# dscripka/openWakeWord

Measured on AMD Instinct MI355X. Metric: real-time audio frames/sec (80 ms frame, 3 wakewords), whole job; real-time streams = value/12.5, higher is better.
Workload: dtype f32 as 3xf16 split MFMA, fp32 accumulate; 1 GPU; 131072 concurrent 16 kHz streams per GPU x 3 heads (alexa,hey_mycroft,hey_jarvis), 80 ms frames, BASELINE configs[3] per-GPU shard; streams_per_gpu=131072, frame_samples=1280, collective=none, gather=none, rccl_ranks=0, pcm_distribution=Gaussian, RMS 3000, pcm=resident in HBM, kernels=mfma_rr_f16x3, graph=False, vad=off, weights=synthetic seed 1234, step_blocks=1

## Files before the change

### openwakeword_amd/csrc/owwhip.hip

```cpp
#include <hip/hip_runtime.h>

#include <algorithm>
#include <cmath>
#include <cstdio>
#include <cstdlib>
#include <cstring>
#include <ctime>
#include <exception>
#include <mutex>
#include <new>
#include <unordered_map>
#include <dlfcn.h>
#include <string>
#include <vector>

#include "owwhip.h"
#include "owwhip_pack.h"
#include "owwhip_ingest.h"
#include "owwhip_mem.h"
#include "owwhip_kernels.h"
#include "owwhip_rr.h"
#include "owwhip_hx.h"
#include "owwhip_vad.h"
#include "owwhip_fused.h"
// ... 90 lines not shown
int stream_create_raw(hipStream_t* s, unsigned flags) { return hipStreamCreateWithFlags(s, flags); }
int stream_destroy_raw(hipStream_t s) { return hipStreamDestroy(s); }
}

namespace {
inline hipError_t herr(int e) { return static_cast<hipError_t>(e); }

hipError_t guard_copy(void* dst, const void* src, size_t n, hipMemcpyKind kind, hipStream_t st) {
    PinnedBuf<char> pin;
    hipError_t e = herr(pin.alloc(n, hipHostMallocDefault));
    if (e != hipSuccess) return e;
    if (kind == hipMemcpyHostToDevice) {
        memcpy(pin, src, n);
        e = hipMemcpyAsync(dst, pin, n, kind, st);
        if (e == hipSuccess) e = hipStreamSynchronize(st);
    } else {
        e = hipMemcpyAsync(pin, src, n, kind, st);
        if (e == hipSuccess) e = hipStreamSynchronize(st);
        if (e == hipSuccess) memcpy(dst, pin, n);
    }
    return e;
}
inline hipError_t copy_async(void* dst, const void* src, size_t n, hipMemcpyKind kind, hipStream_t st) {
    if (guard_mode() && n && (kind == hipMemcpyHostToDevice || kind == hipMemcpyDeviceToHost)) return guard_copy(dst, src, n, kind, st);
    return hipMemcpyAsync(dst, src, n, kind, st);
}
inline hipError_t copy_sync(void* dst, const void* src, size_t n, hipMemcpyKind kind) {
    if (guard_mode() && n && (kind == hipMemcpyHostToDevice || kind == hipMemcpyDeviceToHost)) return guard_copy(dst, src, n, kind, nullptr);
    const hipError_t e = hipMemcpy(dst, src, n, kind);
    return e != hipSuccess || kind != hipMemcpyHostToDevice ? e : hipStreamSynchronize(nullptr);
}

constexpr int kSmallLaunchWgs = 2 * 256;

struct FastGroup : HeadGroup {
    DevBuf<NetDesc> d_nets;
    const float* d_w1pk = nullptr;
    const float* d_b1cat = nullptr;
    const float* d_w1hx = nullptr;
    std::vector<owh::HeadHxNet> hx_net;
};

owh::HeadHxNet make_hx_net(const NetHost& n, int ht, const HxNetPack& p, const float* img, const float* b3, int hx_efeat) {
    const int HP = 16 * ht;
    const float* pd = img + p.pad;
    owh::HeadHxNet o{};
    o.w2hx = img + p.w2; o.b1 = pd; o.ln1g = pd + HP; o.ln1b = pd + 2 * HP; o.b2 = pd + 3 * HP; o.ln2g = pd + 4 * HP; o.ln2b = pd + 5 * HP;
    if (ht == 4) { o.w3 = pd + 6 * HP; o.b3 = b3 ? b3 : pd + 7 * HP; }
    else { o.b3 = pd + 6 * HP; o.w3hx = img + p.w3; o.u3 = std::ldexp(1.0f, -p.e3); }
    o.has_ln = n.has_ln; o.role = n.role; o.head = n.head; o.out_col = n.out_col;
    o.hidden = n.hidden; o.inv_hidden = 1.0f / (float)n.hidden;
    o.u1 = std::ldexp(1.0f, -(hx_efeat + p.e1) + (n.has_ln ? 0 : p.eh)); o.u2 = std::ldexp(1.0f, -(p.e2 + p.eh));
    o.n_out = n.n_out; o.final_act = n.final_act;
    return o;
}

struct EventRec { owm::Event a, b; int cls = 0; };

}

struct oww_ctx : PackIn {
    owm::Stream stream, up_stream, down_stream;
    oww_config cfg{};
    int S = 0, Spad = 0, kmax = 1, TR = 16, NL = 0;
    bool committed = false;
    const int* state_len = kStateLenRr;
// ... 36 lines not shown
    DevBuf<long long> d_prof;
    int prof_block = -1;
    DevBuf<uint32_t> d_nfeat, d_npred, d_nvad;
    DevBuf<float> d_vadring, d_vadin; float vad_threshold = 0.f;
    bool vad = false;
    const float *d_vad_hann = nullptr, *d_vad_encw = nullptr, *d_vad_encb = nullptr, *d_vad_lstmw = nullptr, *d_vad_lstmb = nullptr, *d_vad_wd = nullptr;
    float vad_bd = 0.f, vad_gain = 50.f;
    DevBuf<float> d_vadx, d_vadhc, d_vadlast;
    DevBuf<int16_t> d_tail, d_pcm;
    DevBuf<int16_t> d_long;
    DevBuf<float> d_callmax;
    PinnedBuf<int> h_range;
    int* d_range = nullptr;
    DevBuf<char> d_rs;
    std::vector<float> rs_taps;
    struct Ingest {
        bool ready = false, mixed = false;
        owi::Table tab;
        DevBuf<float> d_taps;
        DevBuf<int16_t> d_hist;
        DevBuf<int16_t> d_out;
        DevBuf<char> d_in;
        DevBuf<uint8_t> d_on;
        DevBuf<IngestClass> d_table;
        DevBuf<uint32_t> d_cls;
        DevBuf<int> d_newcls;
    } ing;
    DevBuf<uint8_t> d_on;
    DevBuf<int> d_lists; PinnedBuf<int> h_lists[2]; owm::Event lists_ev[2]; unsigned lists_turn = 0;
    int k_last = 1;
    float hx_absmax[20] = {};
    std::vector<int16_t> cal_user;
    int small_wgs = kSmallLaunchWgs, small_wgs_heads = kSmallLaunchWgs;
    float hx_selftest_err = 0.f, hx_selftest_ref = 0.f, hx_selftest_score_err = 0.f;
    bool fuse = false;
    DevBuf<float> d_verw, d_verb, d_verthr; DevBuf<int> d_verT;
    int ver_stride = 0, n_verifiers = 0;
    std::vector<int> ver_T;
    bool post_in_heads = false;
    DevBuf<float> d_save;
    DevBuf<int> d_ids;
    DevBuf<int> d_patience;
    DevBuf<float> d_threshold;
    int debounce_frames = 0;
    void* comm = nullptr; int comm_rank = 0, comm_world = 1;
    bool timing = false;
    std::vector<EventRec> ev;
    size_t ev_used = 0;
    double t_ms[OWW_N_KERNEL_CLASSES] = {};
    int64_t t_n[OWW_N_KERNEL_CLASSES] = {};
    bool want_graph = false;
    hipGraph_t graph = nullptr;
    hipGraphExec_t graph_exec = nullptr;
    struct BankHead {
        bool live = false;
        int T = 0, hidden = 0, has_ln = 0, ht = 4, patience = 0;
        float threshold = NAN;
        DevBuf<float> d_img;
        size_t w1_bytes = 0;
        owh::BankHeadDev dev{};
    };
    int bank_K = 0, bank_cap = 0;
    std::vector<BankHead> bank;
    std::vector<int> bank_sub;
    DevBuf<int> d_bank_sub, d_bank_idx;
    DevBuf<float> d_bank_raw, d_bank_scores, d_bank_ring;
// ... 106 lines not shown
        p.prof_block = h->prof_block;
    };
    {
        StageParams p{}; fill(p, h->d_xA, h->d_xB, 3, 2, 3);
        Timed t(h, 2);
        hipLaunchKernelGGL((stage_kernel<CfgB, MFMA, false>), dim3((n_active + CfgB::B - 1) / CfgB::B), dim3(CfgB::NT), CfgB::LDS_BYTES, st, p);
    }
    {
        StageParams p{}; fill(p, h->d_xB, h->d_xC, 7, 4, 5);
        Timed t(h, 3);
        hipLaunchKernelGGL((stage_kernel<CfgC, MFMA, false>), dim3((n_active + CfgC::B - 1) / CfgC::B), dim3(CfgC::NT), CfgC::LDS_BYTES, st, p);
    }
    {
        StageParams p{}; fill(p, h->d_xC, h->d_xD, 11, 6, 7);
        Timed t(h, 4);
        hipLaunchKernelGGL((stage_kernel<CfgD, MFMA, false>), dim3((n_active + CfgD::B - 1) / CfgD::B), dim3(CfgD::NT), CfgD::LDS_BYTES, st, p);
    }
    {
        StageParams p{}; fill(p, h->d_xD, nullptr, 15, 8, 9);
        p.hist19 = h->d_state[10]; p.w19 = h->d_conv[19]; p.feat = h->d_feat; p.emb = h->d_emb; p.nfeat = h->d_nfeat; p.TR = h->TR;
        p.dbg_off[4] = dbg_off[19];
        Timed t(h, 5);
        hipLaunchKernelGGL((stage_kernel<CfgE, MFMA, true>), dim3((n_active + CfgE::B - 1) / CfgE::B), dim3(CfgE::NT), CfgE::LDS_BYTES, st, p);
    }
    HIPCHK(hipGetLastError());
    return 0;
}

template <class CR, class CH, int WG, bool LAST, bool DBG, bool HX>
void launch_rstage(oww_ctx* h, const owr::RStageParams& p, int cls) {
    hipStream_t st = h->stream;
    Timed t(h, cls);
    const int nwg = (p.n_groups + WG - 1) / WG;
    if (HX && !DBG && nwg <= h->small_wgs) hipLaunchKernelGGL((owh::hstage_kernel<CH, LAST, false, WG, 3>), dim3(nwg), dim3(64 * WG), 0, st, p);
    else if (HX) hipLaunchKernelGGL((owh::hstage_kernel<CH, LAST, DBG, WG>), dim3(nwg), dim3(64 * WG), 0, st, p);
    else hipLaunchKernelGGL((owr::rstage_kernel<CR, LAST, DBG>), dim3((p.n_groups + 3) / 4), dim3(256), 0, st, p);
}

template <bool DBG, bool HX>
int run_cnn_rr(oww_ctx* h, const StepArgs& a, int n_active, int mel_stride, int mel_off) {
    using namespace owr;
    hipStream_t st = h->stream;
    int off = 0, dbg_off[20];
    for (int l = 0; l < 20; ++l) { dbg_off[l] = off; off += kLayerOut[l][0] * kLayerOut[l][1] * kLayerOut[l][2]; }
    {
        RAParams p{};
        p.mel = a.mel ? a.mel : h->d_mel; p.mel_stride = mel_stride; p.mel_off = mel_off;
        p.hist_mel = h->d_state[0]; p.hist2 = h->d_state[1];
        p.w0 = h->d_conv[0]; p.w1 = h->d_conv[1]; p.w2 = h->d_conv[2];
        for (int i = 0; i < 3; ++i) { p.scale[i] = h->d_scale[i]; p.shift[i] = h->d_shift[i]; p.dbg_off[i] = dbg_off[i]; }
        p.xout = h->d_xA; p.n_streams = n_active; p.S = h->Spad;
        p.dbg = DBG ? h->d_dbg : nullptr; p.dbg_stride = DBG_FLOATS;
        for (int i = 0; i < 3; ++i) { p.clampv[i] = -0.4f * ldexpf(1.f, h->hx_e[i]); p.dbg_mul[i] = ldexpf(1.f, -h->hx_e[i]); }
        p.xmul = ldexpf(1.f, h->hx_xexp[0]);
        p.range_flag = HX ? h->d_range : nullptr;
        p.stream_on = a.on;
        const int grid = std::min((n_active + 3) / 4, 768);
        Timed t(h, 1);
        if (HX && a.fused_pcm) {
            owf::MelAParams q{};
            q.a = p; q.a.mel = nullptr; q.a.n_streams = h->S;
            q.pcm = a.fused_pcm; q.tail = h->d_tail; q.nfeat = h->d_nfeat; q.hann = h->d_hann; q.mel_start = h->d_mstart; q.mel_taps = h->d_taps; q.mel_off = h->d_meloff; q.mel_dst = h->d_meldst;
            q.mel_out = h->cfg.debug_layers ? h->d_mel : nullptr;
            const int per_cu = std::max(1, std::min(12 / owf::FA_WG, 163840 / owf::FA_LDS_BYTES));
            const int g2 = std::max(1, std::min((q.a.n_streams + owf::FA_WG - 1) / owf::FA_WG, 256 * per_cu));
            hipLaunchKernelGGL(owf::hmelA_kernel<DBG>, dim3(g2), dim3(64 * owf::FA_WG), owf::FA_LDS_BYTES, st, q);
// ... 880 lines not shown
    if (int rc = dalloc(h->stream, h->d_ring, SP * std::max(h->NL, 1) * OWW_SCORE_RING)) return rc;
    if (int rc = dalloc(h->stream, h->d_featinit, (size_t)h->TR * 96)) return rc;
    if (int rc = dalloc(h->stream, h->d_nfeat, SP)) return rc;
    if (int rc = dalloc(h->stream, h->d_npred, SP)) return rc;
    if (int rc = dalloc(h->stream, h->d_vadring, SP * 8)) return rc;
    if (int rc = dalloc(h->stream, h->d_nvad, SP)) return rc;
    if (int rc = dalloc(h->stream, h->d_vadin, SP)) return rc;
    if (h->vad) {
        const size_t G = (SP + 15) / 16;
        if (int rc = dalloc(h->stream, h->d_vadx, G * 4 * 1024)) return rc;
        if (int rc = dalloc(h->stream, h->d_vadhc, G * 4096)) return rc;
        if (int rc = dalloc(h->stream, h->d_vadlast, SP)) return rc;
    }
    if (int rc = dalloc(h->stream, h->d_tail, SP * 480)) return rc;
    if (int rc = dalloc(h->stream, h->d_pcm, (size_t)h->S * OWW_CHUNK * h->kmax)) return rc;
    if (int rc = dalloc(h->stream, h->d_patience, (size_t)std::max(h->NL, 1))) return rc;
    if (int rc = dalloc(h->stream, h->d_threshold, (size_t)std::max(h->NL, 1))) return rc;
    {
        std::vector<float> nanv(std::max(h->NL, 1), NAN);
        HIPCHK(copy_async(h->d_threshold, nanv.data(), nanv.size() * sizeof(float), hipMemcpyHostToDevice, h->stream));
    }
    if (h->cfg.debug_layers) if (int rc = dalloc(h->stream, h->d_dbg, SP * DBG_FLOATS)) return rc;
    if (const char* e = getenv("OWW_PROF_BLOCK")) { h->prof_block = atoi(e); if (int rc = dalloc(h->stream, h->d_prof, (size_t)4 * 256)) return rc; }
    return 0;
}

int set_kernel_lds(oww_ctx* h) {
    int rc = 0;
    auto lds = [&rc](auto kernel, int bytes) { if (!rc) rc = set_lds(kernel, bytes); };
    for (const auto& g : h->groups) if (g.ht == 4) lds(heads64_kernel, heads_lds_bytes(g.NH));
    if (!h->rnn_nets.empty()) lds(heads_rnn_kernel<RNN_SPW>, (int)rnn_lds_bytes(RNN_TMAX));
    if (h->vad) lds(owv::vad_front_kernel, owv::V_LDS_BYTES);
    lds(owf::hmelA_kernel<false>, owf::FA_LDS_BYTES); lds(owf::hmelA_kernel<true>, owf::FA_LDS_BYTES);
    lds(stageA_kernel<true>, CfgA::LDS_BYTES); lds(stageA_kernel<false>, CfgA::LDS_BYTES);
    lds(stage_kernel<CfgB, true, false>, CfgB::LDS_BYTES); lds(stage_kernel<CfgB, false, false>, CfgB::LDS_BYTES);
    lds(stage_kernel<CfgC, true, false>, CfgC::LDS_BYTES); lds(stage_kernel<CfgC, false, false>, CfgC::LDS_BYTES);
    lds(stage_kernel<CfgD, true, false>, CfgD::LDS_BYTES); lds(stage_kernel<CfgD, false, false>, CfgD::LDS_BYTES);
    lds(stage_kernel<CfgE, true, true>, CfgE::LDS_BYTES); lds(stage_kernel<CfgE, false, true>, CfgE::LDS_BYTES);
    return rc;
}

int derive_reset_state(oww_ctx* h, const HxCalib& cal, CommitClock& clk) {
    const size_t SP = h->Spad;
    const int warm = std::min<int>(32, (int)SP);
    hipLaunchKernelGGL(fill_kernel, dim3((warm * 256 + 255) / 256), dim3(256), 0, h->stream, h->d_mel, (size_t)warm * 256, 1.0f);
    const StepArgs args{};
    for (int it = 0; it < 12; ++it)
        if (int rc = run_cnn(h, args, warm, 256, 0)) return rc;
    for (int a = 0; a < N_STATE; ++a)
        HIPCHK(copy_async(h->d_tmpl[a], h->d_state[a], (size_t)h->state_len[a] * (h->rr ? kStateSpgRr[a] : 1) * sizeof(float),
                              hipMemcpyDeviceToDevice, h->stream));
    HIPCHK(hipMemsetAsync(h->d_mel, 0, SP * 8 * h->kmax * 32 * sizeof(float), h->stream));
    HIPCHK(hipMemsetAsync(h->d_emb, 0, SP * 96 * sizeof(float), h->stream));
    if (int rc = do_reset(h, nullptr, (int)SP, nullptr)) return rc;
    HIPCHK(hipStreamSynchronize(h->stream));
    clk.lap("warm-up + reset");
    if (int rc = range_check(h, "oww_commit")) return rc;
    if (h->hx && !getenv("OWW_NO_COMMIT_SELFTEST")) {
        if (int rc = selftest_hx(h, cal)) return rc;
        HIPCHK(hipMemsetAsync(h->d_mel, 0, SP * 8 * h->kmax * 32 * sizeof(float), h->stream));
        HIPCHK(hipMemsetAsync(h->d_emb, 0, SP * 96 * sizeof(float), h->stream));
        HIPCHK(hipMemsetAsync(h->d_raw, 0, SP * std::max(h->NL, 1) * sizeof(float), h->stream));
        if (int rc = do_reset(h, nullptr, (int)SP, nullptr)) return rc;
        HIPCHK(hipStreamSynchronize(h->stream));
        clk.lap("self-test replay + reset");
    }
// ... 344 lines not shown
    if (int rc = build_nets(*h, h->NL, h->TR, h->generic_hmax)) return rc;
    if (h->evt_rows > h->TR)
        return fail(OWW_EINVAL, "oww_events_configure: feature_rows = %d exceeds the handle's feature ring (%d rows)", h->evt_rows, h->TR);
    CommitClock clk(h->hx ? "f16-split" : "family");
    HxCalib cal;
    if (h->hx) {
        if (int rc = calibrate_hx(h, cal)) return rc;
        h->probe_emb = cal.ref_emb; h->probe_nb = cal.nb;
        clk.lap("calibration (total)");
        if (getenv("OWW_DEBUG_CALIB"))
            for (int l = 0; l < 20; ++l) fprintf(stderr, "calib layer %2d: max|a| %-12.5g e_in %4d e_out %4d\n", l, h->hx_absmax[l], h->hx_ein[l], h->hx_e[l]);
    }
    HostBuf hb;
    WeightOff off;
    HeadGroups hg;
    h->no_wide_heads = getenv("OWW_NO_WIDE_HEADS") != nullptr;
    if (int rc = pack_mel_tables(*h, hb, off)) return rc;
    if (int rc = pack_cnn(*h, hb, off)) return rc;
    pack_net_arrays(*h, hb, off);
    if (int rc = pack_head_groups(*h, hg, hb, off)) return rc;
    h->groups.clear();
    for (const HeadGroup& g : hg.groups) h->groups.push_back(FastGroup{g});
    h->generic_nets = hg.generic_nets; h->rnn_nets = hg.rnn_nets;
    h->vad = !h->vad_blob.empty();
    if (int rc = pack_vad(*h, hb, off, h->vad_gain, h->vad_bd)) return rc;
    clk.lap("weight packing (host)");
    if (int rc = bind_weights(h, hb, off)) return rc;
    if (int rc = alloc_range_flag(h)) return rc;
    clk.lap("weight upload");
    if (int rc = alloc_state(h)) return rc;
    h->fuse = h->hx && !getenv("OWW_NO_FUSE");
    if (const char* e = getenv("OWW_SMALL_WGS")) h->small_wgs = atoi(e);
    if (const char* e = getenv("OWW_SMALL_WGS_HEADS")) h->small_wgs_heads = atoi(e);
    if (const char* e = getenv("OWW_GENERIC_SPW")) { const int v = atoi(e); h->generic_spw = v == 4 || v == 16 ? v : 0; }
    h->post_in_heads = h->fuse && h->groups.size() == 1 && h->groups[0].ht == 4 && h->generic_nets.empty() && h->rnn_nets.empty() && h->NL > 0;
    if (int rc = set_kernel_lds(h)) return rc;
    clk.lap("state allocation");
    if (int rc = derive_reset_state(h, cal, clk)) return rc;
    if (h->bank_K > 0) if (int rc = alloc_bank(h)) return rc;
    if (h->vpool_cap > 0) if (int rc = alloc_verifiers(h)) return rc;
    if (events_on(h)) if (int rc = alloc_events(h)) return rc;
    h->committed = true;
    return OWW_OK;
    OWW_GUARD_END
}

int oww_reset(oww_ctx* h, const int32_t* stream_ids, int32_t n, const float* init_features) {
    OWW_GUARD_BEGIN
    if (!h || !h->committed) return fail(OWW_ESTATE, "oww_reset: handle not committed");
    HIPCHK(hipSetDevice(h->cfg.device));
    const float* d_init = nullptr;
    if (init_features) {
        HIPCHK(copy_async(h->d_featinit, init_features, (size_t)h->TR * 96 * sizeof(float), hipMemcpyHostToDevice, h->stream));
        d_init = h->d_featinit;
    }
    if (!stream_ids) {
        if (int rc = do_reset(h, nullptr, h->Spad, d_init)) return rc;
    } else {
        if (n < 1) return OWW_OK;
        for (int i = 0; i < n; ++i)
            if (stream_ids[i] < 0 || stream_ids[i] >= h->S) return fail(OWW_EINVAL, "oww_reset: stream id %d out of range", stream_ids[i]);
        if (int rc = upload_ids(h, stream_ids, n)) return rc;
        if (int rc = do_reset(h, h->d_ids, n, d_init)) return rc;
    }
    if (h->ing.ready && h->ing.tab.Hpad_max) {
        hipLaunchKernelGGL(ingest_hist_reset_kernel, dim3(stream_ids ? n : h->S), dim3(64), 0, h->stream, h->ing.d_hist, h->ing.tab.Hpad_max,
// ... 1451 lines not shown
```

### openwakeword_amd/csrc/owwhip_hx.h

```cpp
#pragma once
#include <type_traits>
#include <utility>
#include "owwhip_layout.h"
#include "owwhip_rr.h"

namespace owh {

using owr::f32x4;
typedef _Float16 f16x8 __attribute__((ext_vector_type(8)));

constexpr float WUNSCALE = 1.0f / 256.0f;

__device__ __forceinline__ float act1(float x, float cl) {
    return fmaxf(fmaxf(0.2f * x, x), cl);
}
template <bool ACT, bool HALF>
__device__ __forceinline__ f32x4 act_t(const f32x4 v, float cl) {
    if (!ACT) return HALF ? f32x4{v[0], v[1], 0.f, 0.f} : v;
    if (HALF) return f32x4{act1(v[0], cl), act1(v[1], cl), 0.f, 0.f};
    return f32x4{act1(v[0], cl), act1(v[1], cl), act1(v[2], cl), act1(v[3], cl)};
}
template <bool HALF>
__device__ __forceinline__ void pin_t(f32x4& v) {
    if (!HALF) { owr::pin(v); return; }
// ... 215 lines not shown
#define OWH_PRICE_HANDOVER 0
#endif
template <bool ON> __device__ __forceinline__ int price_alias(int i) { return ON ? (i & 511) : i; }

template <int N> __device__ __forceinline__ void wait_vmcnt() {
    static_assert(N >= 0 && N < 64, "vmcnt is a 6-bit field");
    __builtin_amdgcn_s_waitcnt((N & 0xF) | ((N >> 4) << 14) | (0x7 << 4) | (0xF << 8));
    asm volatile("" ::: "memory");
}
template <int NS> struct WRing { float* s[5]; };
template <int MAX> __device__ __forceinline__ void wait_vmcnt_of(int n) {
    if (n >= MAX) wait_vmcnt<MAX>();
    else if constexpr (MAX > 0) wait_vmcnt_of<MAX - 1>(n);
}
template <int NBLK, int WG>
__device__ __forceinline__ void issue_chunk_uniform(const float* __restrict__ gsrc, float* ldst, int wave, int lane) {
    const unsigned voff = lane * 4;
#pragma unroll
    for (int u = 0; u < (NBLK + WG - 1) / WG; ++u) {
        const int i = min(u * WG + wave, NBLK - 1);
        const float* base = owr::uniform_ptr(gsrc + i * 256);
        __builtin_amdgcn_global_load_lds((const __attribute__((address_space(1))) void*)(base + voff),
                                         (__attribute__((address_space(3))) void*)(ldst + i * 256), 16, 0, 0);
    }
}
template <int NS, int NBLK, int WG>
__device__ __forceinline__ void ring_issue(const float* __restrict__ gsrc, float* ldst, int wave, int lane) {
    if constexpr (NS == 2) owr::issue_chunk<NBLK, WG>(gsrc, ldst, wave, lane);
    else issue_chunk_uniform<NBLK, WG>(gsrc, ldst, wave, lane);
}
template <int NS, int CH, int NBLK, int NCTO, int NEXT_NBLK, int WG>
__device__ __forceinline__ const float* ring_begin(const WRing<NS>& r, int oct, const float* __restrict__ w, const float* __restrict__ w_next,
                                                   int wave, int lane) {
    constexpr int P = NS - 1;
    const int c = oct + P;
    float* dst = r.s[(CH + oct + P) % NS];
    if (c < NCTO) ring_issue<NS, NBLK, WG>(w + (size_t)c * NBLK * 256, dst, wave, lane);
    else if (NEXT_NBLK > 0 && c - NCTO < P) ring_issue<NS, (NEXT_NBLK > 0 ? NEXT_NBLK : 1), WG>(w_next + (size_t)(c - NCTO) * NEXT_NBLK * 256, dst, wave, lane);
    return r.s[(CH + oct) % NS];
}
template <int NS, int NBLK, int NCTO, int NEXT_NBLK, int WG>
__device__ __forceinline__ void ring_end(int oct) {
    if (!(oct + 1 < NCTO || NEXT_NBLK > 0)) return;
    if constexpr (NS == 2) owr::chunk_sync();
    else {
        constexpr int P = NS - 1, A = (NBLK + WG - 1) / WG, B = NEXT_NBLK > 0 ? ((NEXT_NBLK > 0 ? NEXT_NBLK : 1) + WG - 1) / WG : 0;
        int n = 0;
#pragma unroll
        for (int c = oct + 2; c <= oct + P; ++c) n += c < NCTO ? A : ((NEXT_NBLK > 0 && c - NCTO < P) ? B : 0);
        wait_vmcnt_of<(P - 1) * (A > B ? A : B)>(n);
        asm volatile("s_waitcnt lgkmcnt(0)\n\ts_barrier" ::: "memory");
    }
}

#ifndef OWH_APIPE_B
#define OWH_APIPE_B 0
#endif
#ifndef OWH_APIPE_C
#define OWH_APIPE_C 3
#endif
#ifndef OWH_APIPE_D
#define OWH_APIPE_D 0
#endif
#ifndef OWH_APIPE_E
#define OWH_APIPE_E 1
#endif
struct APair { f16x8 h, l; };
__device__ __forceinline__ APair apair_load(const float* cur, int blk, int lane) { return APair{lds_h(cur, blk, lane), lds_h(cur, blk + 1, lane)}; }
__device__ __forceinline__ void apair_pin(APair& a) {
    typedef unsigned u32x4 __attribute__((ext_vector_type(4)));
    u32x4 x = __builtin_bit_cast(u32x4, a.h), y = __builtin_bit_cast(u32x4, a.l);
    asm volatile("" : "+v"(x), "+v"(y));
    a.h = __builtin_bit_cast(f16x8, x); a.l = __builtin_bit_cast(f16x8, y);
}
__device__ __forceinline__ void apipe_step(APair& curp, APair& nextp, const float* cur, int next_blk, int lane) {
    apair_pin(curp);
    if (next_blk >= 0) nextp = apair_load(cur, next_blk, lane);
// ... 379 lines not shown
            }
#pragma unroll
            for (int r = 0; r < NR; ++r) {
                if (HOUT && oct == NCTO) { out[r][oct - 1] = act_t<BN, true>(prev[r], cl); pin_t<true>(out[r][oct - 1]); }
                else { out[r][oct - 1] = act_t<BN, false>(prev[r], cl); pin_t<false>(out[r][oct - 1]); }
            }
        }
#if OWH_PIPE_M
        if (oct > 0 && oct < NCTO) {
#pragma unroll
            for (int i = 0; i < 3 * (3 * KSF + NMK) * NR; ++i) {
                __builtin_amdgcn_sched_group_barrier(0x008, 1, 0);
                __builtin_amdgcn_sched_group_barrier(0x002, OWH_PIPE_VALU, 0);
            }
        }
#endif
        if (oct < NCTO) {
#pragma unroll
            for (int r = 0; r < NR; ++r) prev[r] = acc[r];
                ring_end<NS, NBLK, NCTO, NEXT_NBLK, WG>(oct);
        }
    }
}

#ifndef OWH_HIST_LDS
#define OWH_HIST_LDS 1
#endif
#ifndef OWH_HIST_LDS_C
#define OWH_HIST_LDS_C 0
#endif
#ifndef OWH_SPRIO_B
#define OWH_SPRIO_B 1111
#endif
#ifndef OWH_SPRIO_C
#define OWH_SPRIO_C 3210
#endif
#ifndef OWH_SPRIO_D
#define OWH_SPRIO_D 3210
#endif
#ifndef OWH_SPRIO_E
#define OWH_SPRIO_E 1111
#endif
template <int CODE, int LAYER> __device__ __forceinline__ void sprio() {
    constexpr int div = LAYER == 0 ? 1000 : LAYER == 1 ? 100 : LAYER == 2 ? 10 : 1;
    if constexpr (CODE != 0 && LAYER >= 0) __builtin_amdgcn_s_setprio((CODE / div) % 10);
    if constexpr (CODE != 0 && LAYER < 0) __builtin_amdgcn_s_setprio(0);
}
template <int NBLK>
__device__ __forceinline__ void issue_hist(const float* __restrict__ gsrc, float* ldst, int lane) {
    const float* base = owr::uniform_ptr(gsrc);
#pragma unroll
    for (int i = 0; i < NBLK; ++i)
        __builtin_amdgcn_global_load_lds((const __attribute__((address_space(1))) void*)(base + i * 256 + lane * 4),
                                         (__attribute__((address_space(3))) void*)(ldst + i * 256), 16, 0, 0);
}
template <int NCT, bool HALF>
__device__ __forceinline__ void load_tile_lds(f32x4 (&t)[NCT], const float* base, int lane) {
#pragma unroll
    for (int ct = 0; ct < NCT; ++ct)
#pragma unroll
        for (int e = 0; e < 4; ++e) {
            if (HALF && ct == NCT - 1 && e >= 2) t[ct][e] = 0.f;
            else t[ct][e] = base[(ct * 4 + e) * 64 + lane];
        }
}

template <class C, bool LAST, bool DBG, int WG = OWH_WG, int NS = 2>
__global__ __launch_bounds__(64 * WG, (DBG || NS > 3 ? 1 : (NS == 3 && C::WPS > 2 ? 2 : C::WPS))) void hstage_kernel(owr::RStageParams p) {
    using namespace owr;
    constexpr int NCTI = C::NCTI, NCT = C::NCT, R = C::RP, F = C::F;
    static_assert(!LAST || C::NPASS == 1, "the last stage runs in one pass");
    static_assert(NS == 2 || C::NPASS == 1 || (4 * NCT) % NS == 0, "multi-pass stages need a ring phase that returns to 0 after each pass");
    static_assert(NS >= 2 && NS <= 5 && NS - 1 <= NCT, "the chunks in flight at a layer boundary belong to at most the next layer");
    constexpr int KSA = (NCTI + 1) / 2, KS = (NCT + 1) / 2;
    constexpr int NBA = 3 * KSA * 2, NB = 3 * KS * 2;
    using TK = TimeK<NCT, C::HOUT>;
    constexpr bool MERGE = OWH_KMERGE && (NCT % 2 == 1) && !LAST && (C::HOUT || OWH_KMERGE_B);
    constexpr int NBT = MERGE ? TK::NBLK : NB;
    constexpr bool PIPE = OWH_PIPE != 0;
    constexpr int APCFG = NCT == 3 ? OWH_APIPE_B : NCT == 5 ? OWH_APIPE_C : LAST ? OWH_APIPE_E : OWH_APIPE_D;
    constexpr bool APM = (APCFG & 1) != 0, APT = (APCFG & 2) != 0;
    constexpr int SPCODE = NCT == 3 ? OWH_SPRIO_B : NCT == 5 ? OWH_SPRIO_C : LAST ? OWH_SPRIO_E : OWH_SPRIO_D;
    constexpr bool REM2 = OWH_REM2 && NCT % 2 == 1 && !C::HOUT && !LAST && !(OWH_KMERGE && OWH_KMERGE_B) && !(OWH_KMERGE_MEL && OWH_KMERGE_MEL2B);
    constexpr bool MMA2 = OWH_KMERGE_MEL && OWH_KMERGE_MEL2 && kInterleave && !C::HIN && NCTI % 2 == 1 && NCTI >= 3 && C::WPS == 2;
    constexpr bool MMA = (OWH_KMERGE_MEL && kInterleave && C::HIN && NCTI % 2 == 1 && NCTI >= 3) || MMA2;
    constexpr int NPRA = MMA2 ? 2 : 1, NMKA = (3 * NPRA + 3) / 4;
    constexpr bool MMC2 = OWH_KMERGE_MEL && OWH_KMERGE_MEL2B && !C::HOUT && NCT % 2 == 1 && NCT >= 3 && !LAST;
    constexpr bool MMC = (OWH_KMERGE_MEL && kInterleave && C::HOUT && NCT % 2 == 1 && NCT >= 3) || MMC2;
    constexpr int NPRC = MMC2 ? 2 : 1, NMKC = (3 * NPRC + 3) / 4;
    constexpr int NBAM = MMA ? (3 * (KSA - 1) + NMKA) * 2 : NBA, NBCM = MMC ? (3 * (KS - 1) + NMKC) * 2 : NB;
    constexpr int NBMAX = (NBAM > NBT ? NBAM : NBT) > (NBCM > (LAST ? NB : 0) ? NBCM : (LAST ? NB : 0)) ? (NBAM > NBT ? NBAM : NBT) : (NBCM > (LAST ? NB : 0) ? NBCM : (LAST ? NB : 0));
    constexpr int WBS = NBMAX * 256;
    constexpr bool HLDS = OWH_HIST_LDS && !LAST && C::NPASS == 1 && (C::SPT == 1 || (C::SPT == 2 && OWH_HIST_LDS_C));
    constexpr int HROW = NCT * 4 * 64;
    const int lane = threadIdx.x & 63;
    const int wave = __builtin_amdgcn_readfirstlane(threadIdx.x >> 6);
    int g = blockIdx.x * WG + wave;
    __shared__ __attribute__((aligned(16))) float wbuf[WBS];
    __shared__ __attribute__((aligned(16))) float wbuf1[WBS];
    __shared__ __attribute__((aligned(16))) float wbuf2[NS >= 3 ? WBS : 4];
    __shared__ __attribute__((aligned(16))) float wbuf3[NS >= 4 ? WBS : 4];
    __shared__ __attribute__((aligned(16))) float wbuf4[NS >= 5 ? WBS : 4];
    const WRing<NS> ring{{wbuf, wbuf1, wbuf2, wbuf3, wbuf4}};
    __shared__ __attribute__((aligned(16))) float sbn[4][NCT * 16];
    __shared__ __attribute__((aligned(16))) float hlds[HLDS ? WG * 2 * HROW : 4];
    float* const hl = hlds + (HLDS ? wave * 2 * HROW : 0);
    const bool active = g < p.n_groups;
    if (!active) g = p.n_groups - 1;
    if (p.glist) g = p.glist[g];
    else g += p.g_base;
    lanemask_t bad = 0;
    ring_issue<NS, NBAM, WG>(p.w[0], wbuf, wave, lane);
    if (NS >= 3) ring_issue<NS, NBAM, WG>(p.w[0] + (size_t)NBAM * 256, wbuf1, wave, lane);
    if (NS >= 4) ring_issue<NS, NBAM, WG>(p.w[0] + (size_t)2 * NBAM * 256, wbuf2, wave, lane);
    if (NS >= 5) ring_issue<NS, NBAM, WG>(p.w[0] + (size_t)3 * NBAM * 256, wbuf3, wave, lane);
    for (int i = threadIdx.x; i < 4 * NCT * 16; i += 64 * WG) {
        const int l = i / (NCT * 16), c = i % (NCT * 16);
        sbn[l][c] = p.shift[l][c];
    }
    const int s_first = g * C::SPT;
    const bool lane_on = active && (p.stream_on == nullptr || p.stream_on[min(s_first + tile_stream<F>(lane & 15), p.S - 1)] != 0);
    float* hb = p.hist_b + (size_t)g * C::HIST_FLOATS;
    float* hd = p.hist_d + (size_t)g * C::HIST_FLOATS;
    if (HLDS) issue_hist<2 * NCT>(hb, hl, lane);

#pragma unroll
    for (int pass = 0; pass < C::NPASS; ++pass) {
    f32x4 Y[R][NCT];
    Op Xo[R][KSA];
#pragma unroll
    for (int r = 0; r < R; ++r) {
        f32x4 X[NCTI];
        load_tile_h<NCTI, C::HIN>(X, p.xin + ((size_t)price_alias<(OWH_PRICE_HANDOVER & 2) != 0 && C::CIN == 24>(g) * C::R + pass * R + r) * (NCTI * 4 * 64), lane);
        to_ops<NCTI, C::HIN>(X, Xo[r]);
    }
    if (pass == 0) chunk_sync();
    sprio<SPCODE, 0>();

    if constexpr (MMA) {
        Op Mx[R][NMKA];
        merge_mel_rems<KSA, R, F, NPRA>(Xo, Mx);
        conv_mel_hxm<KSA, NMKA, NCT, R, F, true, 0, NBT, WG, C::HOUT, NS, APM>(Xo, Mx, Y, ring, p.w[0], p.w[1], sbn[0], p.clampv[0], wave, lane, bad);
    } else
    conv_mel_hx<KSA, NCT, R, F, true, 0, NBT, WG, C::HOUT, false, NS, APM>(Xo, Y, ring, p.w[0], p.w[1], sbn[0], p.clampv[0], wave, lane, bad);
    if (DBG && p.dbg && active) {
#pragma unroll
        for (int r = 0; r < R; ++r) dump_tile_ht<NCT, F, C::C>(Y[r], p.dbg, p.dbg_stride, p.dbg_off[0], s_first, pass * R + r, p.S, lane, p.dbg_mul[0]);
    }
    Op Ao[R][KS], H0[KS], H1[KS];
    sprio<SPCODE, 1>();
    if constexpr (MERGE) {
        Op AoF[R][TK::KSF], H0F[TK::KSF], H1F[TK::KSF], M[R][TK::NMK];
        RemPairs rem[R + 2];
        {
            f32x4 T0[NCT], T1[NCT];
            if (HLDS) { load_tile_lds<NCT, C::HOUT>(T0, hl, lane); load_tile_lds<NCT, C::HOUT>(T1, hl + HROW, lane); }
            else { load_tile_h<NCT, C::HOUT>(T0, hb, lane); load_tile_h<NCT, C::HOUT>(T1, hb + NCT * 4 * 64, lane); }
            to_ops_time<NCT, C::HOUT>(T0, H0F, rem[0]);
            to_ops_time<NCT, C::HOUT>(T1, H1F, rem[1]);
        }
        if (HLDS) { asm volatile("s_waitcnt lgkmcnt(0)" ::: "memory"); issue_hist<2 * NCT>(hd, hl, lane); }
        if (lane_on) {
            store_tile_h<NCT, C::HOUT>(Y[R - 2], hb, lane);
            store_tile_h<NCT, C::HOUT>(Y[R - 1], hb + NCT * 4 * 64, lane);
        }
#pragma unroll
        for (int r = 0; r < R; ++r) to_ops_time<NCT, C::HOUT>(Y[r], AoF[r], rem[2 + r]);
        merge_rems<R, TK::NPR, TK::NMK>(rem, M);
        __builtin_amdgcn_sched_barrier(0);
        conv_time_hxm<TK::KSF, TK::NMK, NCT, R, true, NCT, NBCM, WG, C::HOUT, NS, APT>(H0F, H1F, AoF, M, Y, ring, p.w[1], p.w[2], sbn[1], p.clampv[1], wave, lane, bad);
    } else {
    {
        f32x4 T0[NCT], T1[NCT];
        if (HLDS) { load_tile_lds<NCT, C::HOUT>(T0, hl, lane); load_tile_lds<NCT, C::HOUT>(T1, hl + HROW, lane); }
        else { load_tile_h<NCT, C::HOUT>(T0, hb, lane); load_tile_h<NCT, C::HOUT>(T1, hb + NCT * 4 * 64, lane); }
        to_ops<NCT, C::HOUT, REM2>(T0, H0);
        to_ops<NCT, C::HOUT, REM2>(T1, H1);
    }
    if (HLDS) { asm volatile("s_waitcnt lgkmcnt(0)" ::: "memory"); issue_hist<2 * NCT>(hd, hl, lane); }
    if (lane_on) {
        store_tile_h<NCT, C::HOUT>(Y[R - 2], hb, lane);
        store_tile_h<NCT, C::HOUT>(Y[R - 1], hb + NCT * 4 * 64, lane);
    }
#pragma unroll
    for (int r = 0; r < R; ++r) to_ops<NCT, C::HOUT, REM2>(Y[r], Ao[r]);
    __builtin_amdgcn_sched_barrier(0);
    conv_time_hx<KS, NCT, R, true, NCT, NBCM, WG, true, C::HOUT, PIPE, REM2, NS, APT>(H0, H1, Ao, Y, ring, p.w[1], p.w[2], sbn[1], p.clampv[1], wave, lane, bad);
    }
    if (DBG && p.dbg && active) {
#pragma unroll
        for (int r = 0; r < R; ++r) dump_tile_ht<NCT, F, C::C>(Y[r], p.dbg, p.dbg_stride, p.dbg_off[1], s_first, pass * R + r, p.S, lane, p.dbg_mul[1]);
    }
#pragma unroll
    for (int r = 0; r < R; ++r) to_ops<NCT, C::HOUT, REM2>(Y[r], Ao[r]);
    __builtin_amdgcn_sched_barrier(0);
    sprio<SPCODE, 2>();
    if constexpr (MMC) {
        Op Mc[R][NMKC];
        merge_mel_rems<KS, R, F, NPRC>(Ao, Mc);
        conv_mel_hxm<KS, NMKC, NCT, R, F, true, 2 * NCT, NBT, WG, C::HOUT, NS, APM>(Ao, Mc, Y, ring, p.w[2], p.w[3], sbn[2], p.clampv[2], wave, lane, bad);
    } else
    conv_mel_hx<KS, NCT, R, F, true, 2 * NCT, NBT, WG, C::HOUT, REM2, NS, APM>(Ao, Y, ring, p.w[2], p.w[3], sbn[2], p.clampv[2], wave, lane, bad);
    if (DBG && p.dbg && active) {
#pragma unroll
        for (int r = 0; r < R; ++r) dump_tile_ht<NCT, F, C::C>(Y[r], p.dbg, p.dbg_stride, p.dbg_off[2], s_first, pass * R + r, p.S, lane, p.dbg_mul[2]);
    }
    sprio<SPCODE, 3>();
    if constexpr (MERGE) {
        Op AoF[R][TK::KSF], H0F[TK::KSF], H1F[TK::KSF], M[R][TK::NMK];
        RemPairs rem[R + 2];
        {
            f32x4 T0[NCT], T1[NCT];
            if (HLDS) { load_tile_lds<NCT, C::HOUT>(T0, hl, lane); load_tile_lds<NCT, C::HOUT>(T1, hl + HROW, lane); }
            else { load_tile_h<NCT, C::HOUT>(T0, hd, lane); load_tile_h<NCT, C::HOUT>(T1, hd + NCT * 4 * 64, lane); }
            to_ops_time<NCT, C::HOUT>(T0, H0F, rem[0]);
            to_ops_time<NCT, C::HOUT>(T1, H1F, rem[1]);
        }
        if (lane_on) {
            store_tile_h<NCT, C::HOUT>(Y[R - 2], hd, lane);
            store_tile_h<NCT, C::HOUT>(Y[R - 1], hd + NCT * 4 * 64, lane);
        }
#pragma unroll
        for (int r = 0; r < R; ++r) to_ops_time<NCT, C::HOUT>(Y[r], AoF[r], rem[2 + r]);
        merge_rems<R, TK::NPR, TK::NMK>(rem, M);
        __builtin_amdgcn_sched_barrier(0);
        conv_time_hxm<TK::KSF, TK::NMK, NCT, R, true, 3 * NCT, (C::NPASS > 1 ? NBAM : 0), WG, C::HOUT, NS, APT>(H0F, H1F, AoF, M, Y, ring, p.w[3], p.w[0], sbn[3], p.clampv[3], wave, lane, bad);
    } else {
    {
        f32x4 T0[NCT], T1[NCT];
        if (HLDS) { load_tile_lds<NCT, C::HOUT>(T0, hl, lane); load_tile_lds<NCT, C::HOUT>(T1, hl + HROW, lane); }
        else { load_tile_h<NCT, C::HOUT>(T0, hd, lane); load_tile_h<NCT, C::HOUT>(T1, hd + NCT * 4 * 64, lane); }
        to_ops<NCT, C::HOUT, REM2>(T0, H0);
        to_ops<NCT, C::HOUT, REM2>(T1, H1);
    }
    if (lane_on) {
        store_tile_h<NCT, C::HOUT>(Y[R - 2], hd, lane);
        store_tile_h<NCT, C::HOUT>(Y[R - 1], hd + NCT * 4 * 64, lane);
    }
#pragma unroll
    for (int r = 0; r < R; ++r) to_ops<NCT, C::HOUT, REM2>(Y[r], Ao[r]);
    __builtin_amdgcn_sched_barrier(0);
    conv_time_hx<KS, NCT, R, true, 3 * NCT, (LAST ? NB : (C::NPASS > 1 ? NBAM : 0)), WG, true, C::HOUT, PIPE, REM2, NS, APT>(H0, H1, Ao, Y, ring, p.w[3], LAST ? p.w19 : p.w[0], sbn[3], p.clampv[3], wave, lane, bad);
    }
    if (DBG && p.dbg && active) {
#pragma unroll
        for (int r = 0; r < R; ++r) dump_tile_ht<NCT, F, C::C>(Y[r], p.dbg, p.dbg_stride, p.dbg_off[3], s_first, pass * R + r, p.S, lane, p.dbg_mul[3]);
    }

    sprio<SPCODE, -1>();
    if (!LAST && lane_on) {
        constexpr int FO = C::FO, RO = C::RO;
        constexpr int SPTN = 16 / FO;
        const int pos = lane & 15, j = lane >> 4;
        const int sp = tile_stream<F>(pos), f = tile_mel<F>(pos);
        const int s = g * C::SPT + sp;
        const int gn = s / SPTN, spn = s % SPTN;
        const int posn = tile_pos<FO>(spn, f / 2);
        constexpr int SH = kInterleave ? C::SPT : 1;
#pragma unroll
        for (int ro = 0; ro < R / C::PT; ++ro) {
            float pm[NCT][4];
// ... 31 lines not shown
                Pl[ct][e] = __builtin_bit_cast(float, __builtin_amdgcn_ds_bpermute(src, __builtin_bit_cast(int, m)));
            }
        float* h19 = p.hist19 + (size_t)g * (2 * NCT * 4 * 64);
        f32x4 T0[NCT], T1[NCT];
        Op H0[KS], H1[KS];
        load_tile<NCT>(T0, h19, lane);
        load_tile<NCT>(T1, h19 + NCT * 4 * 64, lane);
        to_ops<NCT>(T0, H0);
        to_ops<NCT>(T1, H1);
        Op Po[1][KS];
        to_ops<NCT>(Pl, Po[0]);
        f32x4 E[1][NCT];
        conv_time_hx<KS, NCT, 1, false, 4 * NCT, 0, WG, false, false, OWH_PIPE != 0, false, NS>(H0, H1, Po, E, ring, p.w19, nullptr, nullptr, 0.f, wave, lane, bad);
        const bool on19 = active && (p.stream_on == nullptr || p.stream_on[min(s_first + (pos & 7), p.S - 1)] != 0);
        if (on19) {
            store_tile<NCT>(T1, h19, lane);
            store_tile<NCT>(Pl, h19 + NCT * 4 * 64, lane);
        }
        const int s = s_first + pos;
        if (on19 && pos < C::SPT && s < p.S) {
            const uint32_t slot = p.nfeat[s] % (uint32_t)p.TR;
#pragma unroll
            for (int ct = 0; ct < NCT; ++ct) {
                const f32x4 ev = E[0][ct] * p.emb_mul;
                *reinterpret_cast<f32x4*>(p.feat + ((size_t)s * p.TR + slot) * 96 + ct * 16 + 4 * j) = ev;
                *reinterpret_cast<f32x4*>(p.emb + (size_t)s * 96 + ct * 16 + 4 * j) = ev;
                if (DBG && p.dbg) *reinterpret_cast<f32x4*>(p.dbg + (size_t)s * p.dbg_stride + p.dbg_off[4] + ct * 16 + 4 * j) = ev;
            }
        }
    }
    }
    if (!LAST && C::NPASS > 1) asm volatile("s_waitcnt vmcnt(0)" ::: "memory");
    raise_range_flag(bad, p.range_flag, s_first, C::SPT);
}

#ifndef OWF_QPRIO
#if !defined(OWF_PRIO) || OWF_PRIO == 6
#define OWF_QPRIO 2233
#else
#define OWF_QPRIO 0
#endif
#endif
namespace sa {
constexpr int RS = 34;
constexpr int PLANE = 344;
constexpr int WAVE_HALVES = 2 * PLANE;
}
typedef unsigned u32x4 __attribute__((ext_vector_type(4)));

__device__ __forceinline__ void stageA_fill_gather_table(int* gtab , int tid, int nt) {
    for (int i = tid; i < 512; i += nt) {
        const int lane = i >> 3, q = i & 7, p = lane & 15, g = lane >> 4, slot = 8 * g + q;
        const int tap = slot % 9, plane = slot >= 18 ? 1 : 0;
        gtab[i] = slot < 27 ? 2 * (plane * sa::PLANE + (tap / 3) * sa::RS + (tap % 3) + 2 * p) : 0;
    }
}
__device__ __forceinline__ void stageA_put_mel(_Float16* sP, int row, int bin, float v) {
    const _Float16 hi = (_Float16)v;
    sP[row * sa::RS + 1 + bin] = hi;
    sP[sa::PLANE + row * sa::RS + 1 + bin] = (_Float16)(v - (float)hi);
}
__device__ __forceinline__ f32x4 mfma3(const f16x8 ah, const f16x8 al, const Op& x, f32x4 c) {
    c = OWH_MFMA(ah, x.h, c);
    c = OWH_MFMA(ah, x.l, c);
    return OWH_MFMA(al, x.h, c);
}
// ... 1132 lines not shown
```

Before: 24.31 million frames/s.

## Add persistent resident-weight variant of stage B hstage kernel

Adds a persistent kernel variant for the HB stage. Each workgroup loads all four layers' weights into 126 KB of dynamic LDS once, then loops over a contiguous range of stream groups using a workgroup-local atomic counter. This replaces the per-group ring streaming of weight chunks from global memory and the chunk syncs between them. It is used by default when there are at least 8192 groups and no group list, with a grid of up to 256 workgroups of 12 waves. The trade-off is one workgroup per CU because of the LDS footprint, and possibly lower occupancy or load imbalance.

New measurement: 24.69 million frames/s (median of 6 runs). 1.02x the previous value.

```diff
diff --git a/openwakeword_amd/csrc/owwhip.hip b/openwakeword_amd/csrc/owwhip.hip
--- a/openwakeword_amd/csrc/owwhip.hip
+++ b/openwakeword_amd/csrc/owwhip.hip
@@ -146,6 +146,8 @@
 }
 
 constexpr int kSmallLaunchWgs = 2 * 256;
+constexpr int kResidentBMinGroups = 8192;
+constexpr int kResidentBWgs = 256;
 
 struct FastGroup : HeadGroup {
     DevBuf<NetDesc> d_nets;
@@ -248,6 +250,7 @@
     float hx_absmax[20] = {};
     std::vector<int16_t> cal_user;
     int small_wgs = kSmallLaunchWgs, small_wgs_heads = kSmallLaunchWgs;
+    int resident_b = -1, resident_b_wgs = kResidentBWgs;
     float hx_selftest_err = 0.f, hx_selftest_ref = 0.f, hx_selftest_score_err = 0.f;
     bool fuse = false;
     DevBuf<float> d_verw, d_verb, d_verthr; DevBuf<int> d_verT;
@@ -420,6 +423,14 @@
     hipStream_t st = h->stream;
     Timed t(h, cls);
     const int nwg = (p.n_groups + WG - 1) / WG;
+    if constexpr (HX && !DBG && std::is_same<CH, owh::HB>::value) {
+        const bool resident = p.glist == nullptr && p.n_groups > 0 && (h->resident_b < 0 ? p.n_groups >= kResidentBMinGroups : h->resident_b != 0);
+        if (resident) {
+            const int grid = std::max(1, std::min(h->resident_b_wgs, (p.n_groups + owh::RES_B_WG - 1) / owh::RES_B_WG));
+            hipLaunchKernelGGL((owh::hstage_kernel<CH, LAST, false, owh::RES_B_WG, 1>), dim3(grid), dim3(64 * owh::RES_B_WG), owh::RES_B_LDS_BYTES, st, p);
+            return;
+        }
+    }
     if (HX && !DBG && nwg <= h->small_wgs) hipLaunchKernelGGL((owh::hstage_kernel<CH, LAST, false, WG, 3>), dim3(nwg), dim3(64 * WG), 0, st, p);
     else if (HX) hipLaunchKernelGGL((owh::hstage_kernel<CH, LAST, DBG, WG>), dim3(nwg), dim3(64 * WG), 0, st, p);
     else hipLaunchKernelGGL((owr::rstage_kernel<CR, LAST, DBG>), dim3((p.n_groups + 3) / 4), dim3(256), 0, st, p);
@@ -1366,6 +1377,7 @@
     if (!h->rnn_nets.empty()) lds(heads_rnn_kernel<RNN_SPW>, (int)rnn_lds_bytes(RNN_TMAX));
     if (h->vad) lds(owv::vad_front_kernel, owv::V_LDS_BYTES);
     lds(owf::hmelA_kernel<false>, owf::FA_LDS_BYTES); lds(owf::hmelA_kernel<true>, owf::FA_LDS_BYTES);
+    lds(owh::hstage_kernel<owh::HB, false, false, owh::RES_B_WG, 1>, owh::RES_B_LDS_BYTES);
     lds(stageA_kernel<true>, CfgA::LDS_BYTES); lds(stageA_kernel<false>, CfgA::LDS_BYTES);
     lds(stage_kernel<CfgB, true, false>, CfgB::LDS_BYTES); lds(stage_kernel<CfgB, false, false>, CfgB::LDS_BYTES);
     lds(stage_kernel<CfgC, true, false>, CfgC::LDS_BYTES); lds(stage_kernel<CfgC, false, false>, CfgC::LDS_BYTES);
@@ -1776,6 +1788,8 @@
     h->fuse = h->hx && !getenv("OWW_NO_FUSE");
     if (const char* e = getenv("OWW_SMALL_WGS")) h->small_wgs = atoi(e);
     if (const char* e = getenv("OWW_SMALL_WGS_HEADS")) h->small_wgs_heads = atoi(e);
+    if (const char* e = getenv("OWW_RESIDENT_B")) h->resident_b = strcmp(e, "auto") == 0 ? -1 : (atoi(e) != 0 ? 1 : 0);
+    if (const char* e = getenv("OWW_RESIDENT_B_WGS")) h->resident_b_wgs = std::max(1, atoi(e));
     if (const char* e = getenv("OWW_GENERIC_SPW")) { const int v = atoi(e); h->generic_spw = v == 4 || v == 16 ? v : 0; }
     h->post_in_heads = h->fuse && h->groups.size() == 1 && h->groups[0].ht == 4 && h->generic_nets.empty() && h->rnn_nets.empty() && h->NL > 0;
     if (int rc = set_kernel_lds(h)) return rc;
diff --git a/openwakeword_amd/csrc/owwhip_hx.h b/openwakeword_amd/csrc/owwhip_hx.h
--- a/openwakeword_amd/csrc/owwhip_hx.h
+++ b/openwakeword_amd/csrc/owwhip_hx.h
@@ -271,17 +271,24 @@
 template <int NS, int CH, int NBLK, int NCTO, int NEXT_NBLK, int WG>
 __device__ __forceinline__ const float* ring_begin(const WRing<NS>& r, int oct, const float* __restrict__ w, const float* __restrict__ w_next,
                                                    int wave, int lane) {
+    if constexpr (NS == 1) {
+        int z = 0;
+        asm volatile("" : "+s"(z));
+        return r.s[CH / NCTO] + oct * NBLK * 256 + z;
+    } else {
     constexpr int P = NS - 1;
     const int c = oct + P;
     float* dst = r.s[(CH + oct + P) % NS];
     if (c < NCTO) ring_issue<NS, NBLK, WG>(w + (size_t)c * NBLK * 256, dst, wave, lane);
     else if (NEXT_NBLK > 0 && c - NCTO < P) ring_issue<NS, (NEXT_NBLK > 0 ? NEXT_NBLK : 1), WG>(w_next + (size_t)(c - NCTO) * NEXT_NBLK * 256, dst, wave, lane);
     return r.s[(CH + oct) % NS];
+    }
 }
 template <int NS, int NBLK, int NCTO, int NEXT_NBLK, int WG>
 __device__ __forceinline__ void ring_end(int oct) {
-    if (!(oct + 1 < NCTO || NEXT_NBLK > 0)) return;
-    if constexpr (NS == 2) owr::chunk_sync();
+    if (NS == 1 || !(oct + 1 < NCTO || NEXT_NBLK > 0)) return;
+    if constexpr (NS == 1) {}
+    else if constexpr (NS == 2) owr::chunk_sync();
     else {
         constexpr int P = NS - 1, A = (NBLK + WG - 1) / WG, B = NEXT_NBLK > 0 ? ((NEXT_NBLK > 0 ? NEXT_NBLK : 1) + WG - 1) / WG : 0;
         int n = 0;
@@ -727,6 +734,12 @@
 #ifndef OWH_SPRIO_B
 #define OWH_SPRIO_B 1111
 #endif
+#ifndef OWH_SPRIO_RB
+#define OWH_SPRIO_RB 1223
+#endif
+#ifndef OWH_RES_HIST_EARLY
+#define OWH_RES_HIST_EARLY 0
+#endif
 #ifndef OWH_SPRIO_C
 #define OWH_SPRIO_C 3210
 #endif
@@ -760,13 +773,20 @@
         }
 }
 
+constexpr int RES_B_WG = 12, RES_B_LDS_BYTES = 126 * 1024;
+template <bool RES> __device__ __forceinline__ float* res_lds(float* ring_slot0) {
+    if constexpr (RES) { extern __shared__ __attribute__((aligned(16))) float res_dyn[]; return res_dyn; }
+    else return ring_slot0;
+}
 template <class C, bool LAST, bool DBG, int WG = OWH_WG, int NS = 2>
-__global__ __launch_bounds__(64 * WG, (DBG || NS > 3 ? 1 : (NS == 3 && C::WPS > 2 ? 2 : C::WPS))) void hstage_kernel(owr::RStageParams p) {
+__global__ __launch_bounds__(64 * WG, (DBG || NS > 3 || NS == 1 ? 1 : (NS == 3 && C::WPS > 2 ? 2 : C::WPS))) void hstage_kernel(owr::RStageParams p) {
     using namespace owr;
     constexpr int NCTI = C::NCTI, NCT = C::NCT, R = C::RP, F = C::F;
     static_assert(!LAST || C::NPASS == 1, "the last stage runs in one pass");
     static_assert(NS == 2 || C::NPASS == 1 || (4 * NCT) % NS == 0, "multi-pass stages need a ring phase that returns to 0 after each pass");
-    static_assert(NS >= 2 && NS <= 5 && NS - 1 <= NCT, "the chunks in flight at a layer boundary belong to at most the next layer");
+    static_assert(NS >= 1 && NS <= 5 && NS - 1 <= NCT, "the chunks in flight at a layer boundary belong to at most the next layer");
+    constexpr bool RES = NS == 1;
+    static_assert(!RES || (!LAST && !DBG && C::NPASS == 1), "resident weights: one pass, no debug dumps, not the last stage");
     constexpr int KSA = (NCTI + 1) / 2, KS = (NCT + 1) / 2;
     constexpr int NBA = 3 * KSA * 2, NB = 3 * KS * 2;
     using TK = TimeK<NCT, C::HOUT>;
@@ -775,7 +795,7 @@
     constexpr bool PIPE = OWH_PIPE != 0;
     constexpr int APCFG = NCT == 3 ? OWH_APIPE_B : NCT == 5 ? OWH_APIPE_C : LAST ? OWH_APIPE_E : OWH_APIPE_D;
     constexpr bool APM = (APCFG & 1) != 0, APT = (APCFG & 2) != 0;
-    constexpr int SPCODE = NCT == 3 ? OWH_SPRIO_B : NCT == 5 ? OWH_SPRIO_C : LAST ? OWH_SPRIO_E : OWH_SPRIO_D;
+    constexpr int SPCODE = NS == 1 ? OWH_SPRIO_RB : NCT == 3 ? OWH_SPRIO_B : NCT == 5 ? OWH_SPRIO_C : LAST ? OWH_SPRIO_E : OWH_SPRIO_D;
     constexpr bool REM2 = OWH_REM2 && NCT % 2 == 1 && !C::HOUT && !LAST && !(OWH_KMERGE && OWH_KMERGE_B) && !(OWH_KMERGE_MEL && OWH_KMERGE_MEL2B);
     constexpr bool MMA2 = OWH_KMERGE_MEL && OWH_KMERGE_MEL2 && kInterleave && !C::HIN && NCTI % 2 == 1 && NCTI >= 3 && C::WPS == 2;
     constexpr bool MMA = (OWH_KMERGE_MEL && kInterleave && C::HIN && NCTI % 2 == 1 && NCTI >= 3) || MMA2;
@@ -786,32 +806,77 @@
     constexpr int NBAM = MMA ? (3 * (KSA - 1) + NMKA) * 2 : NBA, NBCM = MMC ? (3 * (KS - 1) + NMKC) * 2 : NB;
     constexpr int NBMAX = (NBAM > NBT ? NBAM : NBT) > (NBCM > (LAST ? NB : 0) ? NBCM : (LAST ? NB : 0)) ? (NBAM > NBT ? NBAM : NBT) : (NBCM > (LAST ? NB : 0) ? NBCM : (LAST ? NB : 0));
     constexpr int WBS = NBMAX * 256;
-    constexpr bool HLDS = OWH_HIST_LDS && !LAST && C::NPASS == 1 && (C::SPT == 1 || (C::SPT == 2 && OWH_HIST_LDS_C));
+    constexpr bool HLDS = OWH_HIST_LDS && !RES && !LAST && C::NPASS == 1 && (C::SPT == 1 || (C::SPT == 2 && OWH_HIST_LDS_C));
     constexpr int HROW = NCT * 4 * 64;
-    const int lane = threadIdx.x & 63;
+    const int lane0 = threadIdx.x & 63;
     const int wave = __builtin_amdgcn_readfirstlane(threadIdx.x >> 6);
     int g = blockIdx.x * WG + wave;
-    __shared__ __attribute__((aligned(16))) float wbuf[WBS];
-    __shared__ __attribute__((aligned(16))) float wbuf1[WBS];
+    __shared__ __attribute__((aligned(16))) float wbuf[RES ? 4 : WBS];
+    __shared__ __attribute__((aligned(16))) float wbuf1[RES ? 4 : WBS];
     __shared__ __attribute__((aligned(16))) float wbuf2[NS >= 3 ? WBS : 4];
     __shared__ __attribute__((aligned(16))) float wbuf3[NS >= 4 ? WBS : 4];
     __shared__ __attribute__((aligned(16))) float wbuf4[NS >= 5 ? WBS : 4];
-    const WRing<NS> ring{{wbuf, wbuf1, wbuf2, wbuf3, wbuf4}};
+    constexpr int RES_OFF_B = NCT * NBAM * 256, RES_OFF_C = RES_OFF_B + NCT * NBT * 256, RES_OFF_D = RES_OFF_C + NCT * NBCM * 256;
+    static_assert(!RES || (RES_OFF_D + NCT * NBT * 256) * 4 == RES_B_LDS_BYTES, "launch_rstage sizes the dynamic LDS with RES_B_LDS_BYTES");
+    float* const rw = res_lds<RES>(wbuf);
+    const WRing<NS> ring{{rw, RES ? rw + RES_OFF_B : wbuf1, RES ? rw + RES_OFF_C : wbuf2, RES ? rw + RES_OFF_D : wbuf3, wbuf4}};
     __shared__ __attribute__((aligned(16))) float sbn[4][NCT * 16];
     __shared__ __attribute__((aligned(16))) float hlds[HLDS ? WG * 2 * HROW : 4];
     float* const hl = hlds + (HLDS ? wave * 2 * HROW : 0);
-    const bool active = g < p.n_groups;
+    __shared__ int res_next;
+    const bool active = RES || g < p.n_groups;
+    int g_end = 0;
+    if constexpr (RES) {
+        const int nwg = gridDim.x, per = p.n_groups / nwg, rem = p.n_groups % nwg, b = blockIdx.x;
+        const int g_lo = b * per + min(b, rem);
+        g_end = g_lo + per + (b < rem ? 1 : 0);
+        if (threadIdx.x == 0) res_next = g_lo;
+        constexpr int off4[5] = {0, RES_OFF_B / 4, RES_OFF_C / 4, RES_OFF_D / 4, RES_B_LDS_BYTES / 16};
+        constexpr int NT = 64 * WG, MAXU = (off4[2] - off4[1] + NT - 1) / NT;
+        static_assert(off4[1] <= MAXU * NT && off4[3] - off4[2] <= MAXU * NT && off4[4] - off4[3] <= MAXU * NT, "layer b's array is the largest");
+        f32x4 t[4][MAXU];
+#pragma unroll
+        for (int l = 0; l < 4; ++l)
+#pragma unroll
+            for (int u = 0; u < MAXU; ++u) {
+                const int i = threadIdx.x + u * NT;
+                if (i < off4[l + 1] - off4[l]) t[l][u] = reinterpret_cast<const f32x4*>(p.w[l])[i];
+            }
+#pragma unroll
+        for (int l = 0; l < 4; ++l)
+#pragma unroll
+            for (int u = 0; u < MAXU; ++u) {
+                const int i = threadIdx.x + u * NT;
+                if (i < off4[l + 1] - off4[l]) reinterpret_cast<f32x4*>(rw)[off4[l] + i] = t[l][u];
+            }
+    } else {
     if (!active) g = p.n_groups - 1;
     if (p.glist) g = p.glist[g];
     else g += p.g_base;
+    }
     lanemask_t bad = 0;
-    ring_issue<NS, NBAM, WG>(p.w[0], wbuf, wave, lane);
-    if (NS >= 3) ring_issue<NS, NBAM, WG>(p.w[0] + (size_t)NBAM * 256, wbuf1, wave, lane);
-    if (NS >= 4) ring_issue<NS, NBAM, WG>(p.w[0] + (size_t)2 * NBAM * 256, wbuf2, wave, lane);
-    if (NS >= 5) ring_issue<NS, NBAM, WG>(p.w[0] + (size_t)3 * NBAM * 256, wbuf3, wave, lane);
+    if constexpr (!RES) {
+    ring_issue<NS, NBAM, WG>(p.w[0], wbuf, wave, lane0);
+    if (NS >= 3) ring_issue<NS, NBAM, WG>(p.w[0] + (size_t)NBAM * 256, wbuf1, wave, lane0);
+    if (NS >= 4) ring_issue<NS, NBAM, WG>(p.w[0] + (size_t)2 * NBAM * 256, wbuf2, wave, lane0);
+    if (NS >= 5) ring_issue<NS, NBAM, WG>(p.w[0] + (size_t)3 * NBAM * 256, wbuf3, wave, lane0);
+    }
     for (int i = threadIdx.x; i < 4 * NCT * 16; i += 64 * WG) {
         const int l = i / (NCT * 16), c = i % (NCT * 16);
         sbn[l][c] = p.shift[l][c];
+    }
+    if constexpr (RES) __syncthreads();
+    for (;;) {
+    int lane_z = 0;
+    if constexpr (RES) asm volatile("" : "+v"(lane_z));
+    const int lane = RES ? ((lane0 + lane_z) & 63) : lane0;
+    if constexpr (RES) {
+        int k = 0;
+        if (lane0 == 0) k = __hip_atomic_fetch_add(&res_next, 1, __ATOMIC_RELAXED, __HIP_MEMORY_SCOPE_WORKGROUP);
+        g = __builtin_amdgcn_readfirstlane(k);
+        if (g >= g_end) break;
+        g += p.g_base;
+        bad = 0;
     }
     const int s_first = g * C::SPT;
     const bool lane_on = active && (p.stream_on == nullptr || p.stream_on[min(s_first + tile_stream<F>(lane & 15), p.S - 1)] != 0);
@@ -829,7 +894,10 @@
         load_tile_h<NCTI, C::HIN>(X, p.xin + ((size_t)price_alias<(OWH_PRICE_HANDOVER & 2) != 0 && C::CIN == 24>(g) * C::R + pass * R + r) * (NCTI * 4 * 64), lane);
         to_ops<NCTI, C::HIN>(X, Xo[r]);
     }
-    if (pass == 0) chunk_sync();
+    constexpr bool HEARLY = RES && OWH_RES_HIST_EARLY != 0 && !MERGE;
+    f32x4 E0[HEARLY ? NCT : 1], E1[HEARLY ? NCT : 1];
+    if constexpr (HEARLY) { load_tile_h<NCT, C::HOUT>(E0, hb, lane); load_tile_h<NCT, C::HOUT>(E1, hb + NCT * 4 * 64, lane); }
+    if (!RES && pass == 0) chunk_sync();
     sprio<SPCODE, 0>();
 
     if constexpr (MMA) {
@@ -865,7 +933,8 @@
         __builtin_amdgcn_sched_barrier(0);
         conv_time_hxm<TK::KSF, TK::NMK, NCT, R, true, NCT, NBCM, WG, C::HOUT, NS, APT>(H0F, H1F, AoF, M, Y, ring, p.w[1], p.w[2], sbn[1], p.clampv[1], wave, lane, bad);
     } else {
-    {
+    if constexpr (HEARLY) { to_ops<NCT, C::HOUT, REM2>(E0, H0); to_ops<NCT, C::HOUT, REM2>(E1, H1); }
+    else {
         f32x4 T0[NCT], T1[NCT];
         if (HLDS) { load_tile_lds<NCT, C::HOUT>(T0, hl, lane); load_tile_lds<NCT, C::HOUT>(T1, hl + HROW, lane); }
         else { load_tile_h<NCT, C::HOUT>(T0, hb, lane); load_tile_h<NCT, C::HOUT>(T1, hb + NCT * 4 * 64, lane); }
@@ -889,6 +958,7 @@
 #pragma unroll
     for (int r = 0; r < R; ++r) to_ops<NCT, C::HOUT, REM2>(Y[r], Ao[r]);
     __builtin_amdgcn_sched_barrier(0);
+    if constexpr (HEARLY) { load_tile_h<NCT, C::HOUT>(E0, hd, lane); load_tile_h<NCT, C::HOUT>(E1, hd + NCT * 4 * 64, lane); }
     sprio<SPCODE, 2>();
     if constexpr (MMC) {
         Op Mc[R][NMKC];
@@ -921,7 +991,8 @@
         __builtin_amdgcn_sched_barrier(0);
         conv_time_hxm<TK::KSF, TK::NMK, NCT, R, true, 3 * NCT, (C::NPASS > 1 ? NBAM : 0), WG, C::HOUT, NS, APT>(H0F, H1F, AoF, M, Y, ring, p.w[3], p.w[0], sbn[3], p.clampv[3], wave, lane, bad);
     } else {
-    {
+    if constexpr (HEARLY) { to_ops<NCT, C::HOUT, REM2>(E0, H0); to_ops<NCT, C::HOUT, REM2>(E1, H1); }
+    else {
         f32x4 T0[NCT], T1[NCT];
         if (HLDS) { load_tile_lds<NCT, C::HOUT>(T0, hl, lane); load_tile_lds<NCT, C::HOUT>(T1, hl + HROW, lane); }
         else { load_tile_h<NCT, C::HOUT>(T0, hd, lane); load_tile_h<NCT, C::HOUT>(T1, hd + NCT * 4 * 64, lane); }
@@ -1019,6 +1090,8 @@
     }
     if (!LAST && C::NPASS > 1) asm volatile("s_waitcnt vmcnt(0)" ::: "memory");
     raise_range_flag(bad, p.range_flag, s_first, C::SPT);
+    if constexpr (!RES) break;
+    }
 }
 
 #ifndef OWF_QPRIO
```
